# graphdeco-inria/reduced-3dgs

Measured on AMD Instinct MI355X. Metric: train iters/s (fwd+bwd) + Mpix/s render, 500k Gaussians @1600x1062, higher is better.
Workload: dtype f32

## Files before the change

reduced-3dgs_amd/csrc/capi.hip:

```cpp
#include "../../include/r3dgs_rasterizer.h"
#include "../../include/r3dgs_quantised.h"

#include <time.h>

#include <atomic>
#include <random>
#include <chrono>
#include <cmath>
#include <cstddef>
#include <cstdlib>
#include <cstring>
#include <deque>
#include <map>
#include <mutex>
#include <unordered_map>
#include <vector>

#include "common.h"
#include "quant_math.h"

namespace r3 {
int env_int(const char* env, int dflt, int lo, int hi)
{
    const char* v = getenv(env);
// ... 388 lines not shown
            issue_preprocess_color(p, &d->pre, s);
            h.end(kColor, "SH colours", s);
        }
        h.begin(kBinning, s);
        issue_tile_binning(p, d, s);
        h.end(kBinning, "tile binning", s);
        h.begin(kBlendFwd, s);
        issue_blend_forward(p, &d->blend, s);
        h.end(kBlendFwd, "blend forward", s);
    }
}

template <class Block>
void launch_write_args(Block* dst, const Block& v, hipStream_t s);

template <class Hooks>
void issue_backward(const BwdPlan& p, BwdPassArgs* d, const BwdPassArgs& args, hipStream_t s, Hooks& h)
{
    h.begin(kBlendBwd, s);
    if (p.has_pairs) {
        issue_unit_order(p, d, args, s);
        h.begin(kBlendBwdKernel, s);
        issue_blend_backward(p, d, args, s);
        h.end(kBlendBwdKernel, "blend backward kernel", s);
        issue_pair_reduce(p, &d->reduce, s);
    } else {
        launch_write_args(d, args, s);
    }
    h.end(kBlendBwd, "blend backward", s);
    h.begin(kPreBwd, s);
    issue_preprocess_backward(p, &d->pre, s);
    h.end(kPreBwd, "preprocess backward", s);
}

template <class Block>
void launch_write_args(Block* dst, const Block& v, hipStream_t s)
{
    hipLaunchKernelGGL(write_args_kernel<Block>, dim3(1), dim3(256), 0, s, dst, v);
}

template <class Block, class Plan, class IssueFn>
void launch_graph(const CtxKey& key, const Plan& plan, const Block& args, hipStream_t s, IssueFn&& issue)
{
    std::lock_guard<std::mutex> lk(g_ctx_mu);
    GraphCtx& c = g_graphs[key];
    if (!c.exec) {
        try {
            R3_HIP(hipMalloc(&c.d_args, sizeof(Block)));
            hipStream_t cap = capture_stream(key.dev);
            R3_HIP(hipStreamBeginCapture(cap, hipStreamCaptureModeThreadLocal));
            try {
                issue(plan, static_cast<Block*>(c.d_args), args, cap);
            } catch (...) {
                hipGraph_t dead = nullptr;
                (void)hipStreamEndCapture(cap, &dead);
                if (dead) (void)hipGraphDestroy(dead);
                throw;
            }
            R3_HIP(hipStreamEndCapture(cap, &c.graph));
            size_t n_root = 0;
            R3_HIP(hipGraphGetRootNodes(c.graph, nullptr, &n_root));
            if (n_root != 1) throw Error("captured pass graph is not a linear chain");
            R3_HIP(hipGraphGetRootNodes(c.graph, &c.node0, &n_root));
            R3_HIP(hipGraphKernelNodeGetParams(c.node0, &c.node0_params));
            R3_HIP(hipGraphInstantiate(&c.exec, c.graph, nullptr, nullptr, 0));
            c.last_use = ++g_use_clock;
        } catch (...) {
            if (c.graph) (void)hipGraphDestroy(c.graph);
            if (c.d_args) (void)hipFree(c.d_args);
            g_graphs.erase(key);
            throw;
        }
        evict_graphs_locked();
    }
    GraphCtx& ctx = g_graphs[key];
    ctx.last_use = ++g_use_clock;
    Block* dst = static_cast<Block*>(ctx.d_args);
    Block copy = args;
    void* params[2] = {&dst, &copy};
    hipKernelNodeParams kp = ctx.node0_params;
    kp.kernelParams = params;
    kp.extra = nullptr;
    R3_HIP(hipGraphExecKernelNodeSetParams(ctx.exec, ctx.node0, &kp));
    R3_HIP(hipGraphLaunch(ctx.exec, s));
}

struct FwdCall {
    int P;
    const int* D;
    int M;
    const int *coeffsNum, *perBand, *cumSum;
    const float* background;
    int width, height;
    const float *means3D, *shs, *colors_precomp, *opacities, *scales;
    float scale_modifier;
    const float *rotations, *cov3D_precomp, *viewmatrix, *projmatrix, *cam_pos;
    float tan_fovx, tan_fovy;
    float* out_color;
    int* out_touched_pixels;
    float* out_transmittance;
    int* radii;
    int calculate_mean_transmittance, debug;
    hipStream_t stream;
    const float* shs_rest;
    int raw;
    int quantised = 0;
    QuantInputs quant = {};
};

void validate_forward(const FwdCall& c)
{
    if (c.quantised) {
        const QuantInputs& q = c.quant;
        if (!q.xyz || !q.geom_ids || !q.sh_ids || !q.codebooks || !c.viewmatrix || !c.projmatrix || !c.cam_pos || !c.background ||
            !c.out_color)
            throw Error("a required pointer is NULL");
        if (reinterpret_cast<uintptr_t>(q.geom_ids) % 8 || reinterpret_cast<uintptr_t>(q.codebooks) % 16 ||
            reinterpret_cast<uintptr_t>(q.xyz) % (q.xyz_is_half ? 2 : 4))
            throw Error("quantised model: geom_ids must be 8-byte aligned, codebooks 16-byte, xyz to its element");
        if (c.width <= 0 || c.height <= 0) throw Error("image size must be positive");
        if (c.calculate_mean_transmittance && (!c.out_touched_pixels || !c.out_transmittance))
            throw Error("counter mode needs out_touched_pixels and out_transmittance");
        return;
    }
    if (!c.means3D || !c.opacities || !c.viewmatrix || !c.projmatrix || !c.cam_pos || !c.background || !c.out_color)
        throw Error("a required pointer is NULL");
    if (!c.colors_precomp && !c.shs) throw Error("provide SHs or precomputed colours");
    if (!c.cov3D_precomp && (!c.scales || !c.rotations)) throw Error("provide scale/rotation or a precomputed 3D covariance");
    if (!c.colors_precomp && !c.coeffsNum && (c.M < 1 || c.M > 16)) throw Error("SH coefficient count M must be in [1,16]");
    if (!c.colors_precomp && !c.coeffsNum && !c.D) throw Error("per-Gaussian degrees must be provided with SHs");
    if (c.width <= 0 || c.height <= 0) throw Error("image size must be positive");
    if (c.calculate_mean_transmittance && (!c.out_touched_pixels || !c.out_transmittance))
        throw Error("counter mode needs out_touched_pixels and out_transmittance");
}

FwdPlan make_fwd_plan(const FwdCall& c, uint32_t reserve)
{
    static const int color_grid_env = env_int("R3DGS_COLOR_GRID", -1, 0, 1 << 20);
    static const bool generic_env = env_is("R3DGS_DEPTH_SORT", "generic");
    FwdPlan p;
    p.P = c.P;
    p.M = c.M;
    p.W = c.width;
    p.H = c.height;
    p.gx = (c.width + kTile - 1) / kTile;
    p.gy = (c.height + kTile - 1) / kTile;
    p.reserve = reserve;
    p.grid_pairs = grid_pairs_for(reserve);
    p.layout = pair_layout(c.P, (size_t)p.gx * p.gy);
    p.nb = depth_bucket_count((size_t)c.P);
    p.ragged = (c.coeffsNum != nullptr && !c.colors_precomp) ? 1 : 0;
    p.counters = c.calculate_mean_transmittance ? 1 : 0;
    p.color_grid = color_grid_env >= 0 ? color_grid_env : std::min(4096, std::max(512, c.P / 512));
    static const int split0_env = env_int("R3DGS_COLOR_SPLIT0", -1, 0, 100), split1_env = env_int("R3DGS_COLOR_SPLIT1", -1, 0, 100);
    const bool big = c.P > (1 << 20);
    const int split0 = split0_env >= 0 ? split0_env : 25, split1 = split1_env >= 0 ? split1_env : big ? 25 : 45;
    p.color_split[0] = split0;
    p.color_split[1] = split0 + split1 > 100 ? 100 - split0 : split1;
    p.color_split[2] = 100 - p.color_split[0] - p.color_split[1];
    p.generic_depth_sort = (generic_env || c.P >= (1 << 24)) ? 1 : 0;
    p.tight = tight_rects();
    p.raw_params = c.raw ? 1 : 0;
    p.quant = c.quantised ? 1 : 0;
    return p;
}

void fill_fwd_args(FwdPassArgs& a, const FwdPlan& p, const FwdCall& c, const GeomState& g, const BinState* b,
                   const ImageState& img, PassInfo* info_dev, uint64_t ticket, bool fuse_header)
{
    memset(&a, 0, sizeof(a));
    int* radii = c.radii ? c.radii : g.radii_internal;
    FwdInputs& in = a.pre.in;
    in.P = c.P;
    in.M = c.M;
    in.degrees = c.D;
    in.means3D = c.means3D;
    in.scales = c.scales;
    in.rotations = c.rotations;
    in.opacities = c.opacities;
    in.shs = c.shs;
    in.cov3D_precomp = c.cov3D_precomp;
    in.colors_precomp = c.colors_precomp;
    in.coeffs_num = p.ragged ? c.coeffsNum : nullptr;
    in.per_band_count = p.ragged ? c.perBand : nullptr;
    in.cumsum_count = p.ragged ? c.cumSum : nullptr;
    a.shs_rest = c.raw ? c.shs_rest : nullptr;
    if (c.quantised) a.quant = c.quant;
    ViewParams& v = a.pre.view;
    v.view = c.viewmatrix;
    v.proj = c.projmatrix;
    v.campos = c.cam_pos;
    v.bg = c.background;
    v.tan_fovx = c.tan_fovx;
    v.tan_fovy = c.tan_fovy;
    v.W = c.width;
    v.H = c.height;
    v.scale_modifier = c.scale_modifier;
    a.pre.rec = g.rec;
    a.pre.rect = g.rect;
    a.pre.depth_key = g.depth_key;
    a.pre.tiles = g.tiles;
    a.pre.partials = g.partials;
    a.pre.radii = radii;
    a.pre.color_blocks = (c.P + kPreBlockSize - 1) / kPreBlockSize;
    a.pre.tight = p.tight;
    a.pre.sh_ddir = (g_next_forward_trains && !p.ragged && c.shs && !c.colors_precomp) ? g.sh_ddir : nullptr;

    a.header.parts = g.partials;
    a.header.n_parts = (int)pre_partials((size_t)c.P);
    a.header.hdr = g.header;
    a.header.info = info_dev;
    a.header.ticket = (uint32_t)ticket_number(ticket);
    a.header.reserve = p.reserve;
    a.header.stamp_sort = p.generic_depth_sort ? 1 : 0;
    a.header.sh_cache = a.pre.sh_ddir ? 1u : 0u;
    const bool leave_ckpt = g_next_forward_trains && bwd_segments() && !p.counters;
    float4* const ckpt = (b && leave_ckpt) ? b->ckpt : nullptr;
    a.header.ckpt = leave_ckpt ? (uint32_t)bwd_segment_log2() : 0u;
    a.header.ckpt_factor_pct = (uint32_t)bwd_segment_factor_pct();
    a.header.n_tiles = (uint32_t)(p.gx * p.gy);

    DepthArgs& d = a.depth;
    d.P = c.P;
    d.nb = p.nb;
    d.rows = (int)depth_hist_rows((size_t)c.P);
    d.per_block = (int)depth_hist_per_block((size_t)c.P);
    d.fuse_header = fuse_header ? 1 : 0;
    d.key = g.depth_key;
    d.tiles = g.tiles;
    d.hdr = g.header;
    d.info = info_dev;
    d.ticket = (uint32_t)ticket_number(ticket);
    d.ds = g.dsort;
    d.hist_rows = g.hist_rows;
    d.hist_base = g.hist_base;
    d.key_sorted = g.key_sorted;
    d.bucket_id = g.bucket_id;
    d.ovf_key = g.ovf_key;
    d.ovf_id = g.ovf_id;
    d.rect = g.rect;
    d.rec16 = g.rec16;
    d.rec16_b = g.rec16_b;
    d.rect_sorted = g.rect_sorted;
    d.order = g.order;
    d.offsets = g.offsets;
    uint32_t* const block_first = (b && fuse_header && !p.generic_depth_sort) ? b->block_first : nullptr;
    d.block_first = block_first;
    d.block_cap = p.reserve / (uint32_t)kRadixBlock + 2u;

    const PairLayout& l = p.layout;
    const size_t Tn = (size_t)p.gx * p.gy;
    if (b) {
        const uint32_t stride = radix_row_stride(p.reserve);
        EmitArgs& e = a.emit;
        e.P = c.P;
        e.gx = p.gx;
        e.hdr = g.header;
        e.order = g.order;
        e.offsets = g.offsets;
        e.block_first = block_first;
        e.rect = g.rect;
        e.rect_sorted = p.generic_depth_sort ? nullptr : g.rect_sorted;
        e.rec = g.rec;
        e.rank_bits = l.rank_bits;
        e.digit_bits = l.digit_bits;
        e.words_out = b->words_a;
        e.cap = p.reserve;
        e.pair_rank = l.wide == 1 ? b->pair_rank : nullptr;
        e.ranges = img.ranges;
        e.n_tiles = (uint32_t)Tn;
        e.radix_rows = b->radix_rows;
        e.row_stride = stride;
        const char* src = b->words_a;
        for (int k = 0; k < l.passes; k++) {
            char* dst = l.wide ? ((k & 1) ? b->words_a : b->words_b) : ((k & 1) ? b->words_c : b->words_b);
            RadixArgs& r = a.radix[k];
            r.hdr = g.header;
            r.in = src;
            r.out = dst;
            r.ids_out = (l.wide == 2 && k == l.passes - 1) ? b->point_list : nullptr;
            r.cap = p.reserve;
            r.shift = l.rank_bits + k * l.digit_bits;
            r.digit_bits = l.digit_bits;
            r.rank_bits = l.rank_bits;
            r.tile_shift = k * l.digit_bits;
            r.rows = b->radix_rows;
            r.base = b->radix_base;
            r.total = b->radix_total + k * kMaxRadixBins;
            r.row_stride = stride;
            src = dst;
        }
        if (src != sorted_words(*b, l)) throw Error("internal: sorted-word buffer mismatch");
        RangesArgs& t = a.ranges;
        t.hdr = g.header;
        t.sorted = src;
        t.cap = p.reserve;
        t.rank_bits = l.rank_bits;
        t.order = nullptr;
        t.point_list = b->point_list;
        t.ranges = img.ranges;
        t.pair_flag = b->pair_flag;
    }
    BlendFwdArgs& f = a.blend;
    f.ranges = img.ranges;
    f.point_list = b ? b->point_list : nullptr;
    f.rec = g.rec;
    f.W = c.width;
    f.H = c.height;
    f.gx = p.gx;
    f.nblocks = (uint32_t)(p.gx * p.gy * 4);
    f.bg = c.background;
    f.out_color = c.out_color;
// ... 900 lines not shown
```

reduced-3dgs_amd/csrc/common.h:

```cpp
#pragma once
#include <hip/hip_runtime.h>
#include <stddef.h>
#include <stdint.h>

#include <functional>
#include <stdexcept>
#include <string>

#include "gauss_math.h"
#include "param_math.h"

namespace r3 {

constexpr size_t kAlign = 256;
constexpr int kPairGrad = 9;
constexpr int kPieceStride = 9;
constexpr int kAccStride = 12;
constexpr int kPairStride = 12;
static_assert(kAccStride >= 12 && kAccStride % 4 == 0 && kPairStride >= 12 && kPairStride % 4 == 0,
              "the kernels move three float4 per row");

constexpr int kPreBlockSize = 256;
struct PrePartial {
    uint32_t visible;
// ... 413 lines not shown
    uint32_t* depth_key;
    uint32_t* tiles;
    PrePartial* partials;
    int* radii;
    int color_blocks;
    int tight;
    float* sh_ddir;
};
struct HeaderArgs {
    const PrePartial* parts;
    int n_parts;
    GeomHeader* hdr;
    PassInfo* info;
    uint32_t ticket;
    uint32_t reserve;
    uint32_t stamp_sort;
    uint32_t sh_cache;
    uint32_t ckpt;
    uint32_t ckpt_factor_pct, n_tiles;
};
struct DepthArgs {
    int P, nb, rows, per_block;
    int fuse_header;
    const uint32_t* key;
    const uint32_t* tiles;
    GeomHeader* hdr;
    PassInfo* info;
    uint32_t ticket;
    DepthSortScratch* ds;
    unsigned long long* hist_rows;
    uint32_t* hist_base;
    uint32_t* key_sorted;
    uint32_t* bucket_id;
    uint32_t* ovf_key;
    uint32_t* ovf_id;
    const ushort4* rect;
    uint4* rec16;
    uint4* rec16_b;
    ushort4* rect_sorted;
    uint32_t* order;
    uint32_t* offsets;
    uint32_t* block_first;
    uint32_t block_cap;
};
struct EmitArgs {
    int P, gx;
    const GeomHeader* hdr;
    const uint32_t* order;
    const uint32_t* offsets;
    const uint32_t* block_first;
    const ushort4* rect;
    const ushort4* rect_sorted;
    GRec* rec;
    int rank_bits, digit_bits;
    char* words_out;
    uint32_t cap;
    uint32_t* pair_rank;
    uint2* ranges;
    uint32_t n_tiles;
    uint32_t* radix_rows;
    uint32_t row_stride;
};
struct RadixArgs {
    const GeomHeader* hdr;
    const char* in;
    char* out;
    uint32_t* ids_out;
    uint32_t cap;
    int shift, digit_bits;
    int rank_bits, tile_shift;
    uint32_t* rows;
    uint32_t* base;
    uint32_t* total;
    uint32_t row_stride;
};
struct RangesArgs {
    const GeomHeader* hdr;
    const char* sorted;
    uint32_t cap;
    int rank_bits;
    const uint32_t* order;
    uint32_t* point_list;
    uint2* ranges;
    unsigned char* pair_flag;
};
struct BlendFwdArgs {
    const uint2* ranges;
    const uint32_t* point_list;
    const GRec* rec;
    int W, H, gx;
    uint32_t nblocks;
    const float* bg;
    float* out_color;
    float* final_T;
    uint32_t* n_contrib;
    int* touched;
    float* transmittance;
    unsigned long long* quad_masks;
    uint32_t* quad_depth;
    float4* ckpt;
    const GeomHeader* hdr;
};
struct BlendBwdArgs {
    const uint2* ranges;
    const uint32_t* point_list;
    const GRec* rec;
    const float* final_T;
    const uint32_t* n_contrib;
    const float* dL_dpix;
    int W, H, gx;
    uint32_t nblocks;
    const float* bg;
    float* pair_grad;
    unsigned char* pair_flag;
    const unsigned long long* quad_masks;
    uint32_t* tile_order;
    uint32_t units_cap;
    const uint32_t* quad_depth;
    const float4* ckpt;
    const GeomHeader* hdr;
    int segments;
};
struct PairReduceArgs {
    const GeomHeader* hdr;
    const float* pair_grad;
    unsigned char* pair_flag;
    const uint32_t* pair_rank;
    uint32_t rank_mask;
    const uint32_t* order;
    const GRec* rec;
    const uint32_t* tiles;
    float* acc;
    float* wave_part;
    uint32_t stamp0, stamp1;
};
struct PreBwdArgs {
    FwdInputs in;
    ViewParams view;
    const int* radii;
    const GRec* rec;
    const uint32_t* tiles;
    const float* acc;
    const float* wave_part;
    uint32_t stamp0, stamp1;
    const GeomHeader* header;
    float lambda_sh;
    const float* sh_ddir;
    int stagger;
    BwdOutputs out;
    const float* shs_rest;
    float* dL_dsh_rest;
};

struct FwdPassArgs {
    PreArgs pre;
    HeaderArgs header;
    DepthArgs depth;
    EmitArgs emit;
    RadixArgs radix[kMaxRadixPasses];
    RangesArgs ranges;
    BlendFwdArgs blend;
    const float* shs_rest;
    QuantInputs quant;
};
struct BwdPassArgs {
    BlendBwdArgs blend;
    PairReduceArgs reduce;
    PreBwdArgs pre;
};
static_assert(sizeof(FwdPassArgs) <= 3072 && sizeof(BwdPassArgs) <= 3072, "pass blocks travel as by-value kernel arguments");

struct FwdPlan {
    int P, M, W, H, gx, gy;
    uint32_t reserve;
    uint32_t grid_pairs;
    PairLayout layout;
    int nb;
    int ragged, counters;
    int color_grid;
    int color_split[3];
    int generic_depth_sort;
    int tight;
    int raw_params;
    int quant;
};
struct BwdPlan {
    int P, M, W, H, gx, gy;
    uint32_t reserve, grid_pairs;
    uint32_t units_cap;
    PairLayout layout;
    int bwd_ppl;
    int has_pairs;
    int f64_chain;
    int raw_params;
};

enum Stage { kPre = 0, kDepthSort, kBinning, kBlendFwd, kBlendBwd, kPreBwd, kColor, kBlendBwdKernel, kNumStages };

void issue_preprocess_geom(const FwdPlan& p, FwdPassArgs* dst, const FwdPassArgs& v, hipStream_t s);
void issue_preprocess_color(const FwdPlan& p, const PreArgs* a, hipStream_t s);
void launch_mark_visible(int P, const float* means3D, const float* view, bool* present, hipStream_t s);
void launch_activate_params(int P, const float* scaling_raw, const float* rotation_raw, float* scales, float* rotations,
                            hipStream_t s);

void launch_quantised_decode(int P, const int* coeffs, const int* perband, const int* cumsum, const QuantInputs& q, float* xyz,
                             float* features_dc, float* features_rest, float* opacity, float* scaling, float* rotation,
                             int* degrees, hipStream_t s);

void issue_header_reduce(const HeaderArgs* a, hipStream_t s);
void prepare_depth_bucket_sort(int nb);
void issue_depth_sort_and_color(const FwdPlan& p, const FwdPassArgs* a, hipStream_t s);
void run_generic_depth_sort(int P, GeomState& g, hipStream_t s);
void issue_tile_binning(const FwdPlan& p, const FwdPassArgs* a, hipStream_t s);
const char* sorted_words(const BinState& b, const PairLayout& l);
void launch_export_keys(int P, int R, int cap, size_t n_tiles, const BinState& b, const GeomState& g, uint64_t* keys_out,
                        hipStream_t s);
void launch_export_point_list(int count, const uint32_t* point_list, const GeomHeader* hdr, uint32_t* out, hipStream_t s);

void issue_blend_forward(const FwdPlan& p, const BlendFwdArgs* a, hipStream_t s);
void issue_unit_order(const BwdPlan& p, BwdPassArgs* dst, const BwdPassArgs& v, hipStream_t s);
void issue_blend_backward(const BwdPlan& p, BwdPassArgs* dst, const BwdPassArgs& v, hipStream_t s);
void issue_pair_reduce(const BwdPlan& p, const PairReduceArgs* a, hipStream_t s);
void issue_preprocess_backward(const BwdPlan& p, const PreBwdArgs* a, hipStream_t s);

void launch_colour_variance_accumulate(int P, const int* D, int M, int max_sh_deg, const float* means3D,
                                       const float* cam_pos, const float* shs, const int* radii, const int* touched,
                                       const float* transmittance, float* wSum, float* wSumSq, float* mean,
                                       float* variance, float* accum, hipStream_t s);

int env_int(const char* env, int dflt, int lo, int hi);

#if defined(__HIPCC__)
template <class Block>
__device__ __forceinline__ void install_block_from_kernarg(Block* dst, int tid, int nthreads)
{
    static_assert(alignof(Block) == 8 && sizeof(Block) % 4 == 0, "kernarg layout: [dst (8 B)][block]");
#if defined(__HIP_DEVICE_COMPILE__)
    typedef const uint32_t __attribute__((address_space(4))) * KernargWords;
    KernargWords src = (KernargWords)__builtin_amdgcn_kernarg_segment_ptr() + sizeof(Block*) / 4;
    uint32_t* d = reinterpret_cast<uint32_t*>(dst);
    for (uint32_t k = (uint32_t)tid; k < sizeof(Block) / 4; k += (uint32_t)nthreads) d[k] = src[k];
#endif
}
#endif

}
```

reduced-3dgs_amd/csrc/preprocess.hip:

```cpp
#include <cstdlib>
#include <map>
#include <mutex>

#include "depth_sort.h"
#include "quant_math.h"

namespace r3 {

constexpr int kPreBlock = kPreBlockSize;
constexpr int kMaxCoeff = 16;
constexpr int kRowFloats = 3 * kMaxCoeff;
constexpr int kWaveShFloats = 64 * kRowFloats + (64 * kRowFloats) / 32;

template <bool ROWS48>
__device__ __forceinline__ int skew(int e)
{
    if (ROWS48) return e + (int)(((uint32_t)e * 43691u) >> 21);
    return e + (e >> 5);
}

template <bool ROWS48>
struct ShRowLds {
    const float* base;
    int roff;
// ... 69 lines not shown
                    dst[split_lds_index<ROWS48>(f + 2, rl, k0, M)] = v[k].z;
                    dst[split_lds_index<ROWS48>(f + 3, rl, k0, M)] = v[k].w;
                }
            }
        }
    } else {
        for (int f = lane; f < len; f += 64) dst[split_lds_index<ROWS48>(f, rl, k0, M)] = src[f];
    }
}

template <bool ROWS48>
__device__ __forceinline__ void stage_split_rows(const float* __restrict__ dc, const float* __restrict__ rest, int wave_first,
                                                 int nrows, int M, float* dst, int lane)
{
    const int rl = 3 * (M - 1);
    const float* s_dc = dc + 3L * wave_first;
    const int n_dc = 3 * nrows, n_rest = rl * nrows;
    if ((nrows & 3) == 0) {
        stage_split_span<ROWS48, true>(s_dc, n_dc, 3, 0, M, dst, lane);
        if (M > 1) stage_split_span<ROWS48, true>(rest + (long)rl * wave_first, n_rest, rl, 3, M, dst, lane);
    } else {
        stage_split_span<ROWS48, false>(s_dc, n_dc, 3, 0, M, dst, lane);
        if (M > 1) stage_split_span<ROWS48, false>(rest + (long)rl * wave_first, n_rest, rl, 3, M, dst, lane);
    }
}

__device__ __forceinline__ int ragged_offset(int idx, const int* coeffs, const int* perband, const int* cumsum, int* deg)
{
    int off = 0;
    *deg = 0;
    if (idx < cumsum[0]) return idx * coeffs[0];
    *deg = 1;
    off += perband[0] * coeffs[0];
    if (idx < cumsum[1]) return off + (idx - cumsum[0]) * coeffs[1];
    *deg = 2;
    off += perband[1] * coeffs[1];
    if (idx < cumsum[2]) return off + (idx - cumsum[1]) * coeffs[2];
    *deg = 3;
    off += perband[2] * coeffs[2];
    return off + (idx - cumsum[2]) * coeffs[3];
}

template <int COLOR>
__global__ __launch_bounds__(kPreBlock) void preprocess_geom_kernel(FwdPassArgs* dst, FwdPassArgs v)
{
    static_assert(COLOR == 0 || COLOR == 4 || COLOR == 5, "0: activated inputs, 4: raw parameters, 5: codebook ids");
    if (blockIdx.x == 0) install_block_from_kernarg(dst, (int)threadIdx.x, kPreBlock);
    const PreArgs a = v.pre;
    const int tid = threadIdx.x, lane = tid & 63, wave = tid >> 6;
    const int P = a.in.P;
    const int i = blockIdx.x * kPreBlock + tid;
    const bool valid = i < P;
    const Camera cam = load_camera(a.view);

    PreOut o;
    o.radius = 0;
    o.tiles = 0;
    o.tiles_ref = 0;
    o.depth = 0.f;
    if (COLOR == 5) {
        if (valid) {
            float m[3], raw_op, sc[3], rq[4], q[4];
            quant_xyz(v.quant.xyz, v.quant.xyz_is_half, i, m);
            const uint2 gw = reinterpret_cast<const uint2*>(v.quant.geom_ids)[i];
            const uint8_t gid[8] = {(uint8_t)gw.x, (uint8_t)(gw.x >> 8), (uint8_t)(gw.x >> 16), (uint8_t)(gw.x >> 24),
                                    (uint8_t)gw.y, (uint8_t)(gw.y >> 8), (uint8_t)(gw.y >> 16), (uint8_t)(gw.y >> 24)};
            quant_geom(v.quant.codebooks, gid, &raw_op, sc, rq);
            for (int k = 0; k < 3; k++) sc[k] = scale_act(sc[k]);
            quat_act(rq, q);
            preprocess_one(cam, m[0], m[1], m[2], sc, q, nullptr, raw_op, &o, a.tight != 0);
        }
    } else if (valid) {
        const float mx = a.in.means3D[3 * i], my = a.in.means3D[3 * i + 1], mz = a.in.means3D[3 * i + 2];
        float sc[3] = {0.f, 0.f, 0.f}, q[4] = {1.f, 0.f, 0.f, 0.f}, c6[6];
        const float* c6p = nullptr;
        if (a.in.cov3D_precomp) {
            for (int k = 0; k < 6; k++) c6[k] = a.in.cov3D_precomp[6 * i + k];
            c6p = c6;
        } else {
            for (int k = 0; k < 3; k++) sc[k] = a.in.scales[3 * i + k];
            const float4 qv = reinterpret_cast<const float4*>(a.in.rotations)[i];
            q[0] = qv.x;
            q[1] = qv.y;
            q[2] = qv.z;
            q[3] = qv.w;
            if (COLOR == 4) {
                const float rq[4] = {q[0], q[1], q[2], q[3]};
                for (int k = 0; k < 3; k++) sc[k] = scale_act(sc[k]);
                quat_act(rq, q);
            }
        }
        preprocess_one(cam, mx, my, mz, sc, q, c6p, a.in.opacities[i], &o, a.tight != 0);
    }
    if (valid) {
        uint32_t dkey = 0xFFFFFFFFu;
        if (o.radius > 0) {
            GRec r;
            r.x = o.px;
            r.y = o.py;
            r.cA = o.conic[0];
            r.cB = o.conic[1];
            r.cC = o.conic[2];
            r.op = o.opacity;
            r.r = r.g = r.b = 0.f;
            r.rect_min = (uint32_t)o.rmin[0] | ((uint32_t)o.rmin[1] << 16);
            r.width_clamp = (uint32_t)(o.rmax[0] - o.rmin[0]);
            r.pair_start = 0xFFFFFFFFu;
            a.rec[i] = r;
            a.rect[i] = make_ushort4((unsigned short)o.rmin[0], (unsigned short)o.rmin[1], (unsigned short)o.rmax[0],
                                     (unsigned short)o.rmax[1]);
            if (o.tiles > 0) dkey = __float_as_uint(o.depth);
        }
        a.radii[i] = o.radius;
        a.tiles[i] = o.tiles;
        a.depth_key[i] = dkey;
    }
    const unsigned long long vmask = __ballot(o.radius > 0);
    const bool binned = o.tiles > 0;
    const unsigned long long bmask = __ballot(binned);
    uint32_t tsum = o.tiles, rsum = o.tiles_ref;
    uint32_t dmax = binned ? __float_as_uint(o.depth) : 0u, dinv = binned ? ~__float_as_uint(o.depth) : 0u;
    for (int off = 32; off > 0; off >>= 1) {
        tsum += (uint32_t)__shfl_xor((int)tsum, off);
        rsum += (uint32_t)__shfl_xor((int)rsum, off);
        dmax = max(dmax, (uint32_t)__shfl_xor((int)dmax, off));
        dinv = max(dinv, (uint32_t)__shfl_xor((int)dinv, off));
    }
    __shared__ uint32_t s_cnt[kPreBlock / 64][6];
    if (lane == 0) {
        s_cnt[wave][0] = (uint32_t)__popcll(vmask);
        s_cnt[wave][1] = tsum;
        s_cnt[wave][2] = dmax;
        s_cnt[wave][3] = dinv;
        s_cnt[wave][4] = (uint32_t)__popcll(bmask);
        s_cnt[wave][5] = rsum;
    }
    __syncthreads();
    if (tid == 0) {
        PrePartial pp = {0u, 0u, 0u, 0u, 0u, 0u, {0u, 0u}};
        for (int k = 0; k < kPreBlock / 64; k++) {
            pp.visible += s_cnt[k][0];
            pp.num_rendered += s_cnt[k][1];
            pp.depth_max = max(pp.depth_max, s_cnt[k][2]);
            pp.depth_inv_min = max(pp.depth_inv_min, s_cnt[k][3]);
            pp.binned += s_cnt[k][4];
            pp.rendered_ref += s_cnt[k][5];
        }
        a.partials[blockIdx.x] = pp;
    }
}

constexpr size_t kColorLds = sizeof(float) * (kPreBlock / 64) * kWaveShFloats;

__device__ __forceinline__ void store_color(GRec* r, const float* rgb, uint32_t cbits)
{
    r->r = rgb[0];
    r->g = rgb[1];
    r->b = rgb[2];
    if (cbits) r->width_clamp |= cbits << 16;
}

template <bool RAGGED, int BLOCK, bool SPLIT = false>
__device__ __forceinline__ void color_role(const PreArgs& a, char* smem, int first, int last, int wg, int n_wg,
                                           const float* shs_rest = nullptr)
{
    float(*s_sh)[kWaveShFloats] = reinterpret_cast<float(*)[kWaveShFloats]>(smem);
    const int tid = threadIdx.x, lane = tid & 63, wave = tid >> 6;
    const int P = a.in.P, M = a.in.M;
    const bool rows48 = !RAGGED && M == 16;
  for (int blk = first + wg; blk < last; blk += n_wg) {
    const int i = blk * BLOCK + tid;
    const bool valid = i < P;
    const int wave_first = blk * BLOCK + wave * 64;
    const bool vis = valid && a.tiles[i] > 0;
    const bool need_sh = vis && (a.in.colors_precomp == nullptr);

    int deg = 0, roff = 0;
    long span_first = 0;
    int span_len = 0;
    if (a.in.colors_precomp == nullptr) {
        if (RAGGED) {
            const int last_i = min(wave_first + 63, P - 1);
            int d0, dl;
            const int off_first = wave_first < P ? ragged_offset(wave_first, a.in.coeffs_num, a.in.per_band_count, a.in.cumsum_count, &d0) : 0;
            const int off_last = wave_first < P ? ragged_offset(last_i, a.in.coeffs_num, a.in.per_band_count, a.in.cumsum_count, &dl) : 0;
            span_first = 3L * off_first;
            span_len = wave_first < P ? 3 * (off_last + (dl + 1) * (dl + 1) - off_first) : 0;
            if (valid) {
                const int off = ragged_offset(i, a.in.coeffs_num, a.in.per_band_count, a.in.cumsum_count, &deg);
                roff = 3 * (off - off_first);
            }
        } else {
            const int nrows = max(0, min(64, P - wave_first));
            span_first = 3L * M * wave_first;
            span_len = nrows * 3 * M;
            roff = lane * 3 * M;
            if (valid) deg = a.in.degrees[i];
        }
    }
    const bool wave_needs = __ballot(need_sh) != 0ull;
    if (SPLIT) {
        if (wave_needs) {
            const int nrows = max(0, min(64, P - wave_first));
            if (rows48)
                stage_split_rows<true>(a.in.shs, shs_rest, wave_first, nrows, M, s_sh[wave], lane);
            else
                stage_split_rows<false>(a.in.shs, shs_rest, wave_first, nrows, M, s_sh[wave], lane);
        }
    } else if (wave_needs) {
        const float* src = a.in.shs + span_first;
        float* dst = s_sh[wave];
        if (((span_first | span_len) & 3) == 0) {
            const float4* src4 = reinterpret_cast<const float4*>(src);
            if (rows48)
                stage_span<true>(src4, span_len >> 2, dst, lane);
            else
                stage_span<false>(src4, span_len >> 2, dst, lane);
        } else {
            for (int e = lane; e < span_len; e += 64) dst[rows48 ? skew<true>(e) : skew<false>(e)] = src[e];
        }
    }
    __syncthreads();

    if (vis) {
        float rgb[3];
        uint32_t cbits = 0;
        if (need_sh) {
            const float campos[3] = {a.view.campos[0], a.view.campos[1], a.view.campos[2]};
            const float mx = a.in.means3D[3 * i], my = a.in.means3D[3 * i + 1], mz = a.in.means3D[3 * i + 2];
            auto eval = [&](const auto& row) {
                sh_to_rgb(deg, row, mx, my, mz, campos, rgb, &cbits);
                if (!RAGGED && a.sh_ddir && deg > 0) {
                    float d9[9];
                    sh_dir_derivs_at(deg, row, mx, my, mz, campos, d9);
                    float* o = a.sh_ddir + 9 * (size_t)i;
#pragma unroll
                    for (int k = 0; k < 9; k++) o[k] = d9[k];
                }
            };
            if (rows48)
                eval(ShRowLds<true>{s_sh[wave] + 49 * lane, 0});
            else
                eval(ShRowLds<false>{s_sh[wave], roff});
        } else {
            rgb[0] = a.in.colors_precomp[3 * i];
            rgb[1] = a.in.colors_precomp[3 * i + 1];
            rgb[2] = a.in.colors_precomp[3 * i + 2];
        }
        store_color(a.rec + i, rgb, cbits);
    }
    __syncthreads();
  }
}

constexpr int kQuantSpanChunks = (64 * kRowFloats + 15 + 15) / 16 + 1;
constexpr int kQuantSpanWords = 4 * kQuantSpanChunks + (4 * kQuantSpanChunks) / 32 + 1;
constexpr size_t kQuantBooksLds = sizeof(float) * kQuantShBooks * kQuantCentres;
constexpr size_t kQuantColorLds = kQuantBooksLds + sizeof(uint32_t) * (kPreBlock / 64) * kQuantSpanWords;
static_assert(kQuantSpanChunks <= 4 * 64, "four chunks per lane cover a span");

struct ShRowQuantLds {
    const uint8_t* ids;
    int roff;
    const float* books;
    __device__ __forceinline__ float at(int e) const
    {
        const int b = roff + e, w = b >> 2;
        const uint32_t id = ids[((w + (w >> 5)) << 2) | (b & 3)];
        return books[(quant_sh_book(e) << 8) + (int)id];
    }
};

template <int BLOCK>
__device__ __forceinline__ void color_role_quant(const PreArgs& a, const QuantInputs& qi, char* smem, int first, int last, int wg,
                                                 int n_wg)
{
    float* s_books = reinterpret_cast<float*>(smem);
    uint32_t(*s_ids)[kQuantSpanWords] = reinterpret_cast<uint32_t(*)[kQuantSpanWords]>(smem + kQuantBooksLds);
    const int tid = threadIdx.x, lane = tid & 63, wave = tid >> 6;
    const int P = a.in.P;
    if (first + wg < last) {
        const float4* src = reinterpret_cast<const float4*>(qi.codebooks);
        for (int k = tid; k < kQuantShBooks * kQuantCentres / 4; k += BLOCK) reinterpret_cast<float4*>(s_books)[k] = src[k];
    }
    const uintptr_t arr_begin = reinterpret_cast<uintptr_t>(qi.sh_ids);
    const uintptr_t arr_end = arr_begin + (uintptr_t)quant_sh_bytes(a.in.coeffs_num, a.in.per_band_count);
  for (int blk = first + wg; blk < last; blk += n_wg) {
    const int i = blk * BLOCK + tid;
    const bool valid = i < P;
    const int wave_first = blk * BLOCK + wave * 64;
    const bool vis = valid && a.tiles[i] > 0;

    int deg = 0, roff = 0;
    uintptr_t win = 0;
    int nchunks = 0;
    if (wave_first < P) {
        const int last_i = min(wave_first + 63, P - 1);
        int d0, dl;
        const int off_first = quant_ragged_offset(wave_first, a.in.coeffs_num, a.in.per_band_count, a.in.cumsum_count, &d0);
        const int off_last = quant_ragged_offset(last_i, a.in.coeffs_num, a.in.per_band_count, a.in.cumsum_count, &dl);
        const uintptr_t span = arr_begin + 3ull * (uintptr_t)off_first;
        const int span_len = 3 * (off_last + (dl + 1) * (dl + 1) - off_first);
        const int head = (int)(span & 15u);
        win = span - (uintptr_t)head;
        nchunks = (head + span_len + 15) >> 4;
        if (valid) {
            const int off = quant_ragged_offset(i, a.in.coeffs_num, a.in.per_band_count, a.in.cumsum_count, &deg);
            roff = head + 3 * (off - off_first);
        }
    }
    if (__ballot(vis) != 0ull) {
        uint4 v[4];
#pragma unroll
        for (int k = 0; k < 4; k++) {
            const int c = k * 64 + lane;
            v[k] = make_uint4(0u, 0u, 0u, 0u);
            if (c < nchunks) {
                const uintptr_t p = win + 16ull * (uintptr_t)c;
                if (p >= arr_begin && p + 16 <= arr_end) {
                    v[k] = *reinterpret_cast<const uint4*>(p);
                } else {
                    uint32_t w[4] = {0u, 0u, 0u, 0u};
                    for (int b = 0; b < 16; b++) {
                        const uintptr_t q = p + (uintptr_t)b;
                        if (q >= arr_begin && q < arr_end) w[b >> 2] |= (uint32_t)(*reinterpret_cast<const uint8_t*>(q)) << (8 * (b & 3));
                    }
                    v[k] = make_uint4(w[0], w[1], w[2], w[3]);
                }
            }
        }
#pragma unroll
        for (int k = 0; k < 4; k++) {
            const int c = k * 64 + lane;
            if (c < nchunks) {
                const int w = 4 * c;
                uint32_t* d = s_ids[wave] + w + (w >> 5);
                d[0] = v[k].x;
                d[1] = v[k].y;
                d[2] = v[k].z;
                d[3] = v[k].w;
            }
        }
    }
    __syncthreads();

    if (vis) {
        float rgb[3], m[3];
        uint32_t cbits = 0;
        const float campos[3] = {a.view.campos[0], a.view.campos[1], a.view.campos[2]};
        quant_xyz(qi.xyz, qi.xyz_is_half, i, m);
        sh_to_rgb(deg, ShRowQuantLds{reinterpret_cast<const uint8_t*>(s_ids[wave]), roff, s_books}, m[0], m[1], m[2], campos, rgb,
                  &cbits);
        store_color(a.rec + i, rgb, cbits);
    }
    __syncthreads();
  }
}

template <bool RAGGED, int BLOCK>
__global__ __launch_bounds__(BLOCK) void preprocess_color_kernel(const PreArgs* __restrict__ ap)
{
    extern __shared__ __attribute__((aligned(16))) char smem[];
    const PreArgs a = *ap;
    color_role<RAGGED, BLOCK>(a, smem, 0, (a.in.P + BLOCK - 1) / BLOCK, (int)blockIdx.x, (int)gridDim.x);
}

template <int BLOCK>
__global__ __launch_bounds__(BLOCK) void preprocess_color_params_kernel(const FwdPassArgs* __restrict__ pa)
{
    extern __shared__ __attribute__((aligned(16))) char smem[];
    const PreArgs a = pa->pre;
    color_role<false, BLOCK, true>(a, smem, 0, (a.in.P + BLOCK - 1) / BLOCK, (int)blockIdx.x, (int)gridDim.x, pa->shs_rest);
}

template <int BLOCK>
__global__ __launch_bounds__(BLOCK) void preprocess_color_quant_kernel(const FwdPassArgs* __restrict__ pa)
{
    extern __shared__ __attribute__((aligned(16))) char smem[];
    const PreArgs a = pa->pre;
    const QuantInputs qi = pa->quant;
    color_role_quant<BLOCK>(a, qi, smem, 0, (a.in.P + BLOCK - 1) / BLOCK, (int)blockIdx.x, (int)gridDim.x);
}

template <int STEP, bool RAGGED>
__global__ __launch_bounds__(kPreBlock) void depth_sort_color_kernel(const FwdPassArgs* __restrict__ pa, int n_sort,
                                                                     int c0, int c1)
{
    extern __shared__ __attribute__((aligned(16))) char smem[];
    const int wg = (int)blockIdx.x;
    if (wg < n_sort) {
        const DepthArgs d = pa->depth;
        if (STEP == 0)
            depth_hist_role(d, pa->header, smem, wg);
        else if (STEP == 1)
            depth_scatter_role(d, smem, wg);
        else
            depth_bucket_group_role(d, smem, wg, n_sort);
    } else {
        const PreArgs a = pa->pre;
        color_role<RAGGED, kPreBlock>(a, smem, c0, c1, wg - n_sort, (int)gridDim.x - n_sort);
    }
}

template <int STEP>
__global__ __launch_bounds__(kPreBlock) void depth_sort_color_params_kernel(const FwdPassArgs* __restrict__ pa, int n_sort,
                                                                            int c0, int c1)
{
    extern __shared__ __attribute__((aligned(16))) char smem[];
    const int wg = (int)blockIdx.x;
    if (wg < n_sort) {
        const DepthArgs d = pa->depth;
        if (STEP == 0)
            depth_hist_role(d, pa->header, smem, wg);
        else if (STEP == 1)
            depth_scatter_role(d, smem, wg);
        else
            depth_bucket_group_role(d, smem, wg, n_sort);
    } else {
        const PreArgs a = pa->pre;
        color_role<false, kPreBlock, true>(a, smem, c0, c1, wg - n_sort, (int)gridDim.x - n_sort, pa->shs_rest);
    }
}

template <int STEP>
__global__ __launch_bounds__(kPreBlock) void depth_sort_color_quant_kernel(const FwdPassArgs* __restrict__ pa, int n_sort,
                                                                           int c0, int c1)
{
    extern __shared__ __attribute__((aligned(16))) char smem[];
    const int wg = (int)blockIdx.x;
    if (wg < n_sort) {
        const DepthArgs d = pa->depth;
        if (STEP == 0)
            depth_hist_role(d, pa->header, smem, wg);
        else if (STEP == 1)
            depth_scatter_role(d, smem, wg);
        else
            depth_bucket_group_role(d, smem, wg, n_sort);
    } else {
        const PreArgs a = pa->pre;
        const QuantInputs qi = pa->quant;
        color_role_quant<kPreBlock>(a, qi, smem, c0, c1, wg - n_sort, (int)gridDim.x - n_sort);
    }
}

__global__ __launch_bounds__(64 * kColWaves) void depth_colscan_kernel(const DepthArgs* __restrict__ ap)
{
    const DepthArgs d = *ap;
    depth_colscan_role(d, (int)blockIdx.x);
}

void issue_preprocess_geom(const FwdPlan& p, FwdPassArgs* dst, const FwdPassArgs& v, hipStream_t s)
{
    const int blocks = (p.P + kPreBlock - 1) / kPreBlock;
    if (p.quant)
        hipLaunchKernelGGL(preprocess_geom_kernel<5>, dim3(blocks), dim3(kPreBlock), 0, s, dst, v);
    else if (p.raw_params)
        hipLaunchKernelGGL(preprocess_geom_kernel<4>, dim3(blocks), dim3(kPreBlock), 0, s, dst, v);
    else
        hipLaunchKernelGGL(preprocess_geom_kernel<0>, dim3(blocks), dim3(kPreBlock), 0, s, dst, v);
}

struct ColorSource {
    void (*sort_step[3])(const FwdPassArgs*, int, int, int);
    const void* color;
    size_t color_lds;
};

static const ColorSource kColorSources[4] = {
    {{depth_sort_color_kernel<0, false>, depth_sort_color_kernel<1, false>, depth_sort_color_kernel<2, false>},
     reinterpret_cast<const void*>(preprocess_color_kernel<false, kPreBlock>), kColorLds},
    {{depth_sort_color_kernel<0, true>, depth_sort_color_kernel<1, true>, depth_sort_color_kernel<2, true>},
     reinterpret_cast<const void*>(preprocess_color_kernel<true, kPreBlock>), kColorLds},
    {{depth_sort_color_params_kernel<0>, depth_sort_color_params_kernel<1>, depth_sort_color_params_kernel<2>},
     reinterpret_cast<const void*>(preprocess_color_params_kernel<kPreBlock>), kColorLds},
    {{depth_sort_color_quant_kernel<0>, depth_sort_color_quant_kernel<1>, depth_sort_color_quant_kernel<2>},
     reinterpret_cast<const void*>(preprocess_color_quant_kernel<kPreBlock>), kQuantColorLds},
};

static const ColorSource& color_source(const FwdPlan& p)
{
    return kColorSources[p.quant ? 3 : p.raw_params ? 2 : p.ragged ? 1 : 0];
}

void issue_preprocess_color(const FwdPlan& p, const PreArgs* a, hipStream_t s)
{
    const int blocks = (p.P + kPreBlock - 1) / kPreBlock;
    const int grid = p.color_grid > 0 && blocks > p.color_grid ? p.color_grid : blocks;
    const ColorSource& src = color_source(p);
    void* args[] = {&a};
    (void)hipLaunchKernel(src.color, dim3(grid), dim3(kPreBlock), args, src.color_lds, s);
}

static size_t max_sz(size_t a, size_t b) { return a > b ? a : b; }

static void opt_in_lds(const void* kernel, size_t bytes)
{
    if (bytes > 48 * 1024) R3_HIP(hipFuncSetAttribute(kernel, hipFuncAttributeMaxDynamicSharedMemorySize, (int)bytes));
}

void prepare_depth_bucket_sort(int nb)
{
    static std::mutex mu;
    static std::map<int, int> prepared;
    std::lock_guard<std::mutex> lk(mu);
    int dev = 0;
    R3_HIP(hipGetDevice(&dev));
    int& prepared_nb = prepared[dev];
    if (nb <= prepared_nb) return;
    const size_t sort_lds[3] = {depth_hist_lds(nb), depth_scatter_lds(nb), kBucketSortLds};
    for (const ColorSource& src : kColorSources) {
        for (int k = 0; k < 3; k++)
            opt_in_lds(reinterpret_cast<const void*>(src.sort_step[k]), max_sz(sort_lds[k], src.color_lds));
        opt_in_lds(src.color, src.color_lds);
    }
    prepared_nb = nb;
}

void issue_depth_sort_and_color(const FwdPlan& p, const FwdPassArgs* pa, hipStream_t s)
{
    const int rows = (int)depth_hist_rows((size_t)p.P), nb = p.nb;
    const int chunks = (p.P + kPreBlock - 1) / kPreBlock;
    int c[4] = {0, 0, 0, chunks};
    c[1] = (int)((long long)chunks * p.color_split[0] / 100);
    c[2] = c[1] + (int)((long long)chunks * p.color_split[1] / 100);
    const int cw = p.color_grid > 0 ? p.color_grid : 512;
    const ColorSource& src = color_source(p);
    const int n_sort[3] = {rows, rows, (nb + kBucketsPerGroup - 1) / kBucketsPerGroup};
    const size_t sort_lds[3] = {depth_hist_lds(nb), depth_scatter_lds(nb), kBucketSortLds};
    auto step = [&](int k) {
        const int n_color = c[k + 1] - c[k] < cw ? c[k + 1] - c[k] : cw;
        const size_t lds = n_color ? max_sz(sort_lds[k], src.color_lds) : sort_lds[k];
        hipLaunchKernelGGL(src.sort_step[k], dim3(n_sort[k] + n_color), dim3(kPreBlock), lds, s, pa, n_sort[k], c[k], c[k + 1]);
    };
    step(0);
    hipLaunchKernelGGL(depth_colscan_kernel, dim3((nb + 1 + 63) / 64), dim3(64 * kColWaves), 0, s, &pa->depth);
    step(1);
    step(2);
}

__global__ __launch_bounds__(256) void mark_visible_kernel(int P, const float* means, const float* view, bool* present)
{
    const int i = blockIdx.x * 256 + threadIdx.x;
    if (i >= P) return;
    float pv[3];
    xform4x3(view, means[3 * i], means[3 * i + 1], means[3 * i + 2], pv);
    present[i] = pv[2] > 0.2f;
}

void launch_mark_visible(int P, const float* means3D, const float* view, bool* present, hipStream_t s)
{
    hipLaunchKernelGGL(mark_visible_kernel, dim3((P + 255) / 256), dim3(256), 0, s, P, means3D, view, present);
}

__global__ __launch_bounds__(256) void activate_params_kernel(int P, const float* __restrict__ scaling_raw,
                                                              const float* __restrict__ rotation_raw,
                                                              float* __restrict__ scales, float* __restrict__ rotations)
{
    const int i = blockIdx.x * 256 + threadIdx.x;
    if (i >= P) return;
    if (scaling_raw && scales)
        for (int k = 0; k < 3; k++) scales[3 * (size_t)i + k] = scale_act(scaling_raw[3 * (size_t)i + k]);
    if (rotation_raw && rotations) {
        const float4 qv = reinterpret_cast<const float4*>(rotation_raw)[i];
        const float rq[4] = {qv.x, qv.y, qv.z, qv.w};
        float q[4];
        quat_act(rq, q);
        reinterpret_cast<float4*>(rotations)[i] = make_float4(q[0], q[1], q[2], q[3]);
    }
}

void launch_activate_params(int P, const float* scaling_raw, const float* rotation_raw, float* scales, float* rotations,
                            hipStream_t s)
{
    hipLaunchKernelGGL(activate_params_kernel, dim3((P + 255) / 256), dim3(256), 0, s, P, scaling_raw, rotation_raw, scales,
                       rotations);
}

__global__ __launch_bounds__(256) void quantised_decode_kernel(int P, const int* __restrict__ coeffs, const int* __restrict__ perband,
                                                               const int* __restrict__ cumsum, QuantInputs q, float* xyz,
                                                               float* features_dc, float* features_rest, float* opacity,
                                                               float* scaling, float* rotation, int* degrees)
{
    const int i = blockIdx.x * 256 + threadIdx.x;
    if (i >= P) return;
    quant_decode_one(i, coeffs, perband, cumsum, q.xyz, q.xyz_is_half, q.geom_ids, q.sh_ids, q.codebooks, xyz, features_dc,
                     features_rest, opacity, scaling, rotation, degrees);
}

void launch_quantised_decode(int P, const int* coeffs, const int* perband, const int* cumsum, const QuantInputs& q, float* xyz,
                             float* features_dc, float* features_rest, float* opacity, float* scaling, float* rotation,
                             int* degrees, hipStream_t s)
{
    hipLaunchKernelGGL(quantised_decode_kernel, dim3((P + 255) / 256), dim3(256), 0, s, P, coeffs, perband, cumsum, q, xyz,
                       features_dc, features_rest, opacity, scaling, rotation, degrees);
}

}
```

Measured before the change: 1576.

## Replace fixed colour split with atomic chunk queue fed alongside sort steps

Drops the static percentage split of colour-evaluation blocks across the three depth-sort launches. Co-resident colour workgroups now pull 64-point wave chunks from a shared atomic counter, and stop taking work in steps 0 and 1 once all sort workgroups have signalled completion. Block-wide barriers in the colour role become wave-level syncs, so each wave runs independently. This should balance the load between sort and colour work dynamically, at the cost of atomic traffic per chunk and a dependence on the queue counters being zeroed before each pass.

After: 900.0. 0.571x the previous value.

```diff
diff --git a/reduced-3dgs_amd/csrc/capi.hip b/reduced-3dgs_amd/csrc/capi.hip
--- a/reduced-3dgs_amd/csrc/capi.hip
+++ b/reduced-3dgs_amd/csrc/capi.hip
@@ -564,12 +564,6 @@
     p.ragged = (c.coeffsNum != nullptr && !c.colors_precomp) ? 1 : 0;
     p.counters = c.calculate_mean_transmittance ? 1 : 0;
     p.color_grid = color_grid_env >= 0 ? color_grid_env : std::min(4096, std::max(512, c.P / 512));
-    static const int split0_env = env_int("R3DGS_COLOR_SPLIT0", -1, 0, 100), split1_env = env_int("R3DGS_COLOR_SPLIT1", -1, 0, 100);
-    const bool big = c.P > (1 << 20);
-    const int split0 = split0_env >= 0 ? split0_env : 25, split1 = split1_env >= 0 ? split1_env : big ? 25 : 45;
-    p.color_split[0] = split0;
-    p.color_split[1] = split0 + split1 > 100 ? 100 - split0 : split1;
-    p.color_split[2] = 100 - p.color_split[0] - p.color_split[1];
     p.generic_depth_sort = (generic_env || c.P >= (1 << 24)) ? 1 : 0;
     p.tight = tight_rects();
     p.raw_params = c.raw ? 1 : 0;
diff --git a/reduced-3dgs_amd/csrc/common.h b/reduced-3dgs_amd/csrc/common.h
--- a/reduced-3dgs_amd/csrc/common.h
+++ b/reduced-3dgs_amd/csrc/common.h
@@ -589,6 +589,12 @@
     float* dL_dsh_rest;
 };
 
+struct ColorQueue {
+    uint32_t next;
+    uint32_t sort_done[2];
+    uint32_t pad;
+};
+
 struct FwdPassArgs {
     PreArgs pre;
     HeaderArgs header;
@@ -599,6 +605,7 @@
     BlendFwdArgs blend;
     const float* shs_rest;
     QuantInputs quant;
+    ColorQueue cq;
 };
 struct BwdPassArgs {
     BlendBwdArgs blend;
@@ -615,7 +622,6 @@
     int nb;
     int ragged, counters;
     int color_grid;
-    int color_split[3];
     int generic_depth_sort;
     int tight;
     int raw_params;
diff --git a/reduced-3dgs_amd/csrc/preprocess.hip b/reduced-3dgs_amd/csrc/preprocess.hip
--- a/reduced-3dgs_amd/csrc/preprocess.hip
+++ b/reduced-3dgs_amd/csrc/preprocess.hip
@@ -245,6 +245,56 @@
 
 constexpr size_t kColorLds = sizeof(float) * (kPreBlock / 64) * kWaveShFloats;
 
+struct ChunkFeed {
+    uint32_t* next;
+    const uint32_t* done;
+    uint32_t n_sort;
+    int cur, stride;
+    int n;
+};
+
+__device__ __forceinline__ ChunkFeed static_feed(int P, int wg, int n_wg, int waves)
+{
+    const int wave = __builtin_amdgcn_readfirstlane((int)(threadIdx.x >> 6));
+    return ChunkFeed{nullptr, nullptr, 0u, wg * waves + wave, n_wg * waves, (P + 63) / 64};
+}
+
+template <int STEP>
+__device__ __forceinline__ ChunkFeed queue_feed(const FwdPassArgs* pa, int P, int n_sort)
+{
+    ColorQueue* q = const_cast<ColorQueue*>(&pa->cq);
+    return ChunkFeed{&q->next, STEP < 2 ? &q->sort_done[STEP] : nullptr, (uint32_t)n_sort, 0, 0, (P + 63) / 64};
+}
+
+__device__ __forceinline__ int take_chunk(ChunkFeed& f, int lane)
+{
+    if (!f.next) {
+        const int c = f.cur;
+        f.cur += f.stride;
+        return c < f.n ? c : -1;
+    }
+    uint32_t c = 0xFFFFFFFFu;
+    if (lane == 0) {
+        const bool over = f.done && __hip_atomic_load(f.done, __ATOMIC_RELAXED, __HIP_MEMORY_SCOPE_AGENT) >= f.n_sort;
+        if (!over) c = atomicAdd(f.next, 1u);
+    }
+    c = (uint32_t)__builtin_amdgcn_readfirstlane((int)c);
+    return c < (uint32_t)f.n ? (int)c : -1;
+}
+
+template <int STEP>
+__device__ __forceinline__ void sort_role_done(const FwdPassArgs* pa)
+{
+    if (STEP < 2 && threadIdx.x == 0) atomicAdd(&const_cast<ColorQueue*>(&pa->cq)->sort_done[STEP], 1u);
+}
+
+__device__ __forceinline__ void wave_window_sync()
+{
+    __builtin_amdgcn_fence(__ATOMIC_RELEASE, "wavefront");
+    __builtin_amdgcn_wave_barrier();
+    __builtin_amdgcn_fence(__ATOMIC_ACQUIRE, "wavefront");
+}
+
 __device__ __forceinline__ void store_color(GRec* r, const float* rgb, uint32_t cbits)
 {
     r->r = rgb[0];
@@ -253,18 +303,17 @@
     if (cbits) r->width_clamp |= cbits << 16;
 }
 
-template <bool RAGGED, int BLOCK, bool SPLIT = false>
-__device__ __forceinline__ void color_role(const PreArgs& a, char* smem, int first, int last, int wg, int n_wg,
-                                           const float* shs_rest = nullptr)
+template <bool RAGGED, bool SPLIT = false>
+__device__ __forceinline__ void color_role(const PreArgs& a, char* smem, ChunkFeed feed, const float* shs_rest = nullptr)
 {
     float(*s_sh)[kWaveShFloats] = reinterpret_cast<float(*)[kWaveShFloats]>(smem);
     const int tid = threadIdx.x, lane = tid & 63, wave = tid >> 6;
     const int P = a.in.P, M = a.in.M;
     const bool rows48 = !RAGGED && M == 16;
-  for (int blk = first + wg; blk < last; blk += n_wg) {
-    const int i = blk * BLOCK + tid;
+  for (int chunk = take_chunk(feed, lane); chunk >= 0; chunk = take_chunk(feed, lane)) {
+    const int wave_first = chunk * 64;
+    const int i = wave_first + lane;
     const bool valid = i < P;
-    const int wave_first = blk * BLOCK + wave * 64;
     const bool vis = valid && a.tiles[i] > 0;
     const bool need_sh = vis && (a.in.colors_precomp == nullptr);
 
@@ -313,7 +362,7 @@
             for (int e = lane; e < span_len; e += 64) dst[rows48 ? skew<true>(e) : skew<false>(e)] = src[e];
         }
     }
-    __syncthreads();
+    wave_window_sync();
 
     if (vis) {
         float rgb[3];
@@ -342,7 +391,7 @@
         }
         store_color(a.rec + i, rgb, cbits);
     }
-    __syncthreads();
+    wave_window_sync();
   }
 }
 
@@ -365,23 +414,23 @@
 };
 
 template <int BLOCK>
-__device__ __forceinline__ void color_role_quant(const PreArgs& a, const QuantInputs& qi, char* smem, int first, int last, int wg,
-                                                 int n_wg)
+__device__ __forceinline__ void color_role_quant(const PreArgs& a, const QuantInputs& qi, char* smem, ChunkFeed feed)
 {
     float* s_books = reinterpret_cast<float*>(smem);
     uint32_t(*s_ids)[kQuantSpanWords] = reinterpret_cast<uint32_t(*)[kQuantSpanWords]>(smem + kQuantBooksLds);
     const int tid = threadIdx.x, lane = tid & 63, wave = tid >> 6;
     const int P = a.in.P;
-    if (first + wg < last) {
+    {
         const float4* src = reinterpret_cast<const float4*>(qi.codebooks);
         for (int k = tid; k < kQuantShBooks * kQuantCentres / 4; k += BLOCK) reinterpret_cast<float4*>(s_books)[k] = src[k];
     }
+    __syncthreads();
     const uintptr_t arr_begin = reinterpret_cast<uintptr_t>(qi.sh_ids);
     const uintptr_t arr_end = arr_begin + (uintptr_t)quant_sh_bytes(a.in.coeffs_num, a.in.per_band_count);
-  for (int blk = first + wg; blk < last; blk += n_wg) {
-    const int i = blk * BLOCK + tid;
+  for (int chunk = take_chunk(feed, lane); chunk >= 0; chunk = take_chunk(feed, lane)) {
+    const int wave_first = chunk * 64;
+    const int i = wave_first + lane;
     const bool valid = i < P;
-    const int wave_first = blk * BLOCK + wave * 64;
     const bool vis = valid && a.tiles[i] > 0;
 
     int deg = 0, roff = 0;
@@ -435,7 +484,7 @@
             }
         }
     }
-    __syncthreads();
+    wave_window_sync();
 
     if (vis) {
         float rgb[3], m[3];
@@ -446,7 +495,7 @@
                   &cbits);
         store_color(a.rec + i, rgb, cbits);
     }
-    __syncthreads();
+    wave_window_sync();
   }
 }
 
@@ -455,7 +504,7 @@
 {
     extern __shared__ __attribute__((aligned(16))) char smem[];
     const PreArgs a = *ap;
-    color_role<RAGGED, BLOCK>(a, smem, 0, (a.in.P + BLOCK - 1) / BLOCK, (int)blockIdx.x, (int)gridDim.x);
+    color_role<RAGGED>(a, smem, static_feed(a.in.P, (int)blockIdx.x, (int)gridDim.x, BLOCK / 64));
 }
 
 template <int BLOCK>
@@ -463,7 +512,7 @@
 {
     extern __shared__ __attribute__((aligned(16))) char smem[];
     const PreArgs a = pa->pre;
-    color_role<false, BLOCK, true>(a, smem, 0, (a.in.P + BLOCK - 1) / BLOCK, (int)blockIdx.x, (int)gridDim.x, pa->shs_rest);
+    color_role<false, true>(a, smem, static_feed(a.in.P, (int)blockIdx.x, (int)gridDim.x, BLOCK / 64), pa->shs_rest);
 }
 
 template <int BLOCK>
@@ -472,12 +521,11 @@
     extern __shared__ __attribute__((aligned(16))) char smem[];
     const PreArgs a = pa->pre;
     const QuantInputs qi = pa->quant;
-    color_role_quant<BLOCK>(a, qi, smem, 0, (a.in.P + BLOCK - 1) / BLOCK, (int)blockIdx.x, (int)gridDim.x);
+    color_role_quant<BLOCK>(a, qi, smem, static_feed(a.in.P, (int)blockIdx.x, (int)gridDim.x, BLOCK / 64));
 }
 
 template <int STEP, bool RAGGED>
-__global__ __launch_bounds__(kPreBlock) void depth_sort_color_kernel(const FwdPassArgs* __restrict__ pa, int n_sort,
-                                                                     int c0, int c1)
+__global__ __launch_bounds__(kPreBlock) void depth_sort_color_kernel(const FwdPassArgs* __restrict__ pa, int n_sort)
 {
     extern __shared__ __attribute__((aligned(16))) char smem[];
     const int wg = (int)blockIdx.x;
@@ -489,15 +537,15 @@
             depth_scatter_role(d, smem, wg);
         else
             depth_bucket_group_role(d, smem, wg, n_sort);
+        sort_role_done<STEP>(pa);
     } else {
         const PreArgs a = pa->pre;
-        color_role<RAGGED, kPreBlock>(a, smem, c0, c1, wg - n_sort, (int)gridDim.x - n_sort);
+        color_role<RAGGED>(a, smem, queue_feed<STEP>(pa, a.in.P, n_sort));
     }
 }
 
 template <int STEP>
-__global__ __launch_bounds__(kPreBlock) void depth_sort_color_params_kernel(const FwdPassArgs* __restrict__ pa, int n_sort,
-                                                                            int c0, int c1)
+__global__ __launch_bounds__(kPreBlock) void depth_sort_color_params_kernel(const FwdPassArgs* __restrict__ pa, int n_sort)
 {
     extern __shared__ __attribute__((aligned(16))) char smem[];
     const int wg = (int)blockIdx.x;
@@ -509,15 +557,15 @@
             depth_scatter_role(d, smem, wg);
         else
             depth_bucket_group_role(d, smem, wg, n_sort);
+        sort_role_done<STEP>(pa);
     } else {
         const PreArgs a = pa->pre;
-        color_role<false, kPreBlock, true>(a, smem, c0, c1, wg - n_sort, (int)gridDim.x - n_sort, pa->shs_rest);
+        color_role<false, true>(a, smem, queue_feed<STEP>(pa, a.in.P, n_sort), pa->shs_rest);
     }
 }
 
 template <int STEP>
-__global__ __launch_bounds__(kPreBlock) void depth_sort_color_quant_kernel(const FwdPassArgs* __restrict__ pa, int n_sort,
-                                                                           int c0, int c1)
+__global__ __launch_bounds__(kPreBlock) void depth_sort_color_quant_kernel(const FwdPassArgs* __restrict__ pa, int n_sort)
 {
     extern __shared__ __attribute__((aligned(16))) char smem[];
     const int wg = (int)blockIdx.x;
@@ -529,10 +577,11 @@
             depth_scatter_role(d, smem, wg);
         else
             depth_bucket_group_role(d, smem, wg, n_sort);
+        sort_role_done<STEP>(pa);
     } else {
         const PreArgs a = pa->pre;
         const QuantInputs qi = pa->quant;
-        color_role_quant<kPreBlock>(a, qi, smem, c0, c1, wg - n_sort, (int)gridDim.x - n_sort);
+        color_role_quant<kPreBlock>(a, qi, smem, queue_feed<STEP>(pa, a.in.P, n_sort));
     }
 }
 
@@ -554,7 +603,7 @@
 }
 
 struct ColorSource {
-    void (*sort_step[3])(const FwdPassArgs*, int, int, int);
+    void (*sort_step[3])(const FwdPassArgs*, int);
     const void* color;
     size_t color_lds;
 };
@@ -612,18 +661,15 @@
 void issue_depth_sort_and_color(const FwdPlan& p, const FwdPassArgs* pa, hipStream_t s)
 {
     const int rows = (int)depth_hist_rows((size_t)p.P), nb = p.nb;
-    const int chunks = (p.P + kPreBlock - 1) / kPreBlock;
-    int c[4] = {0, 0, 0, chunks};
-    c[1] = (int)((long long)chunks * p.color_split[0] / 100);
-    c[2] = c[1] + (int)((long long)chunks * p.color_split[1] / 100);
+    const int chunks = (p.P + 63) / 64, wg_chunks = (chunks + kPreBlock / 64 - 1) / (kPreBlock / 64);
     const int cw = p.color_grid > 0 ? p.color_grid : 512;
+    const int n_color = wg_chunks < cw ? wg_chunks : cw;
     const ColorSource& src = color_source(p);
     const int n_sort[3] = {rows, rows, (nb + kBucketsPerGroup - 1) / kBucketsPerGroup};
     const size_t sort_lds[3] = {depth_hist_lds(nb), depth_scatter_lds(nb), kBucketSortLds};
     auto step = [&](int k) {
-        const int n_color = c[k + 1] - c[k] < cw ? c[k + 1] - c[k] : cw;
         const size_t lds = n_color ? max_sz(sort_lds[k], src.color_lds) : sort_lds[k];
-        hipLaunchKernelGGL(src.sort_step[k], dim3(n_sort[k] + n_color), dim3(kPreBlock), lds, s, pa, n_sort[k], c[k], c[k + 1]);
+        hipLaunchKernelGGL(src.sort_step[k], dim3(n_sort[k] + n_color), dim3(kPreBlock), lds, s, pa, n_sort[k]);
     };
     step(0);
     hipLaunchKernelGGL(depth_colscan_kernel, dim3((nb + 1 + 63) / 64), dim3(64 * kColWaves), 0, s, &pa->depth);
```
